# Keep-Passion/ImageStitch

Hardware: AMD Instinct MI355X
Metric: image-pairs/sec (2048x2048 grayscale, SURF+BF) (higher is better)
Workload: dtype f32

## Files before the change

### imagestitch_amd/_lib.py

```python
import ctypes as C
import os

import numpy as np

_HERE = os.path.dirname(os.path.abspath(__file__))
LIB_PATH = os.path.abspath(os.environ["VFSMS_LIB"]) if os.environ.get("VFSMS_LIB") else os.path.join(_HERE, "lib", "libvfsms.so")

VFSMS_OK = 0
VFSMS_ERR_BAD_ARG, VFSMS_ERR_CAPACITY, VFSMS_ERR_UNSUPPORTED = -1, -2, -6
ATTEMPT_INTS = 8


class VfsmsError(RuntimeError):
    pass


class SurfParams(C.Structure):
    _fields_ = [("hessian_threshold", C.c_float), ("n_octaves", C.c_int32), ("n_octave_layers", C.c_int32),
                ("extended", C.c_int32), ("upright", C.c_int32)]


class OrbParams(C.Structure):
    _fields_ = [("n_features", C.c_int32), ("scale_factor", C.c_float), ("n_levels", C.c_int32), ("edge_threshold", C.c_int32),
                ("first_level", C.c_int32), ("wta_k", C.c_int32), ("score_type", C.c_int32), ("patch_size", C.c_int32),
# ... 42 lines not shown
    "vfsms_ctx_sync": (C.c_int, [C.c_void_p]),
    "vfsms_ctx_sync_uploads": (C.c_int, [C.c_void_p]),
    "vfsms_ctx_stream": (C.c_void_p, [C.c_void_p]),
    "vfsms_ctx_set_keypoint_capacity": (C.c_int, [C.c_void_p, C.c_int]),
    "vfsms_ctx_set_offset_estimator": (C.c_int, [C.c_void_p, C.c_int, C.c_int]),
    "vfsms_ctx_set_offset_verifier": (C.c_int, [C.c_void_p, C.c_int, C.c_double, C.c_int]),
    "vfsms_ctx_set_phase_resolver": (C.c_int, [C.c_void_p, C.c_int, C.c_int, C.c_double, C.c_int]),
    "vfsms_attempt_phase_resolve_batch": (C.c_int, [C.c_void_p, C.POINTER(RoiPair), C.c_int, C.c_int, C.c_double, C.c_int, C.c_void_p, C.c_void_p, C.c_void_p]),
    "vfsms_phase_resolve_u8": (C.c_int, [C.c_void_p, C.c_void_p, C.c_void_p, C.c_int, C.c_int, C.c_int, C.c_int, C.c_int, C.c_double, C.c_int,
                                         C.c_void_p, C.c_void_p, C.c_void_p]),
    "vfsms_verify_ncc": (C.c_int, [C.c_void_p, C.c_void_p, C.c_int, C.c_void_p, C.c_int, C.c_int, C.c_int, C.c_int, C.c_int, C.c_int, C.c_void_p]),
    "vfsms_ncc_search_batch": (C.c_int, [C.c_void_p, C.POINTER(NccJob), C.c_int, C.c_int, C.c_int, C.c_void_p, C.c_void_p]),
    "vfsms_profile_enable": (C.c_int, [C.c_void_p, C.c_int]),
    "vfsms_profile_read": (C.c_int, [C.c_void_p, C.c_char_p, C.c_int, C.c_void_p, C.c_void_p, C.c_int, C.POINTER(C.c_int), C.c_int]),
    "vfsms_tile_upload": (C.c_int, [C.c_void_p, C.c_void_p, C.c_int, C.c_int, C.c_int, C.POINTER(C.c_int64)]),
    "vfsms_tile_upload_async": (C.c_int, [C.c_void_p, C.c_void_p, C.c_int, C.c_int, C.c_int, C.POINTER(C.c_int64)]),
    "vfsms_tile_reserve": (C.c_int, [C.c_void_p, C.c_int, C.c_int, C.POINTER(C.c_int64)]),
    "vfsms_tile_fill": (C.c_int, [C.c_void_p, C.c_int64, C.c_void_p, C.c_int]),
    "vfsms_tile_reserve_ch": (C.c_int, [C.c_void_p, C.c_int, C.c_int, C.c_int, C.POINTER(C.c_int64)]),
    "vfsms_tile_fill_pair": (C.c_int, [C.c_void_p, C.c_int64, C.c_int64, C.c_void_p, C.c_int, C.c_int]),
    "vfsms_tile_fill_jpeg": (C.c_int, [C.c_void_p, C.c_int64, C.c_int64, C.c_char_p, C.c_size_t]),
    "vfsms_jpeg_decode": (C.c_int, [C.c_char_p, C.c_size_t, C.c_int, C.c_void_p, C.c_size_t, C.POINTER(C.c_int), C.POINTER(C.c_int), C.POINTER(C.c_int)]),
    "vfsms_jpeg_encode": (C.c_int, [C.c_void_p, C.c_int, C.c_int, C.c_int, C.c_int, C.c_int, C.c_int, C.c_void_p, C.c_size_t, C.POINTER(C.c_size_t)]),
    "vfsms_jpeg_header": (C.c_int, [C.c_int, C.c_int, C.c_int, C.c_int, C.c_int, C.c_void_p, C.c_size_t, C.POINTER(C.c_size_t)]),
    "vfsms_jpeg_encode_device": (C.c_int, [C.c_void_p, C.c_void_p, C.c_int, C.c_int, C.c_int, C.c_int, C.c_int, C.c_int, C.c_int, C.c_void_p, C.c_size_t, C.POINTER(C.c_size_t)]),
    "vfsms_canvas_encode_jpeg_rows": (C.c_int, [C.c_void_p, C.c_int64, C.c_int, C.c_int, C.c_int, C.c_int, C.c_void_p, C.c_size_t, C.POINTER(C.c_size_t)]),
    "vfsms_jpeg_join": (C.c_int, [C.POINTER(C.c_void_p), C.POINTER(C.c_size_t), C.c_int, C.c_int, C.c_int, C.c_void_p, C.c_size_t, C.POINTER(C.c_size_t)]),
    "vfsms_canvas_blend_tile_resident": (C.c_int, [C.c_void_p, C.c_int64, C.c_int64, C.c_int, C.c_int, C.c_int, C.c_int, C.c_int, C.c_int, C.c_int]),
    "vfsms_host_alloc": (C.c_int, [C.c_void_p, C.c_size_t, C.POINTER(C.c_void_p)]),
    "vfsms_host_free": (C.c_int, [C.c_void_p, C.c_void_p]),
    "vfsms_tile_wrap": (C.c_int, [C.c_void_p, C.c_void_p, C.c_int, C.c_int, C.c_int, C.POINTER(C.c_int64)]),
    "vfsms_tile_free": (C.c_int, [C.c_void_p, C.c_int64]),
    "vfsms_integral_u8_i32": (C.c_int, [C.c_void_p, C.c_void_p, C.c_int, C.c_int, C.c_int, C.c_void_p]),
    "vfsms_surf_detect_describe": (C.c_int, [C.c_void_p, C.c_void_p, C.c_int, C.c_int, C.c_int, C.POINTER(SurfParams),
                                             C.c_void_p, C.c_void_p, C.c_void_p, C.c_int, C.POINTER(C.c_int)]),
    "vfsms_surf_detect": (C.c_int, [C.c_void_p, C.c_void_p, C.c_int, C.c_int, C.c_int, C.POINTER(SurfParams),
                                    C.c_void_p, C.c_int, C.POINTER(C.c_int)]),
    "vfsms_orb_detect_describe": (C.c_int, [C.c_void_p, C.c_void_p, C.c_int, C.c_int, C.c_int, C.POINTER(OrbParams),
                                            C.c_void_p, C.c_void_p, C.c_void_p, C.c_int, C.POINTER(C.c_int)]),
    "vfsms_sift_detect_describe": (C.c_int, [C.c_void_p, C.c_void_p, C.c_int, C.c_int, C.c_int, C.POINTER(SiftParams),
                                             C.c_void_p, C.c_void_p, C.c_void_p, C.c_int, C.POINTER(C.c_int)]),
    "vfsms_sift_pyramid": (C.c_int, [C.c_void_p, C.c_void_p, C.c_int, C.c_int, C.c_int, C.POINTER(SiftParams),
                                     C.c_void_p, C.c_void_p, C.c_size_t, C.c_void_p, C.c_int, C.POINTER(C.c_int)]),
    "vfsms_attempt_orb_batch": (C.c_int, [C.c_void_p, C.POINTER(RoiPair), C.c_int, C.POINTER(OrbParams), C.c_int, C.c_int, C.c_void_p]),
    "vfsms_attempt_sift_batch": (C.c_int, [C.c_void_p, C.POINTER(RoiPair), C.c_int, C.POINTER(SiftParams), C.c_double, C.c_int, C.c_void_p]),
    "vfsms_bf_l2_knn2_ratio": (C.c_int, [C.c_void_p, C.c_void_p, C.c_int, C.c_void_p, C.c_int, C.c_int, C.c_double,
                                         C.c_void_p, C.c_int, C.POINTER(C.c_int)]),
    "vfsms_bf_l2_knn2": (C.c_int, [C.c_void_p, C.c_void_p, C.c_int, C.c_void_p, C.c_int, C.c_int,
                                   C.c_void_p, C.c_void_p, C.c_void_p]),
    "vfsms_bf_hamming_nn": (C.c_int, [C.c_void_p, C.c_void_p, C.c_int, C.c_void_p, C.c_int, C.c_int, C.c_int,
                                      C.c_void_p, C.c_int, C.POINTER(C.c_int)]),
    "vfsms_mode_offset": (C.c_int, [C.c_void_p, C.c_void_p, C.c_int, C.c_void_p, C.c_int, C.c_void_p, C.c_int,
                                    C.c_int, C.c_void_p]),
    "vfsms_consensus_offset": (C.c_int, [C.c_void_p, C.c_void_p, C.c_int, C.c_void_p, C.c_int, C.c_void_p, C.c_int,
                                         C.c_int, C.c_int, C.c_void_p]),
    "vfsms_phase_correlate_u8": (C.c_int, [C.c_void_p, C.c_void_p, C.c_void_p, C.c_int, C.c_int, C.c_int, C.c_int,
                                           C.c_void_p]),
    "vfsms_fuse_fade_i64": (C.c_int, [C.c_void_p, C.c_void_p, C.c_void_p, C.c_int, C.c_int, C.c_int, C.c_int, C.c_int,
                                      C.c_void_p, C.c_void_p]),
    "vfsms_fuse_ramps_i64": (C.c_int, [C.c_void_p, C.c_void_p, C.c_int, C.c_int, C.c_int, C.c_int, C.c_int, C.c_int,
                                       C.c_void_p, C.c_void_p]),
    "vfsms_attempt_surf_batch": (C.c_int, [C.c_void_p, C.POINTER(RoiPair), C.c_int, C.POINTER(SurfParams), C.c_double,
                                           C.c_int, C.c_void_p]),
    "vfsms_attempt_surf_batch_enhanced": (C.c_int, [C.c_void_p, C.POINTER(RoiPair), C.c_int, C.POINTER(SurfParams), C.c_double,
                                                    C.c_int, C.c_int, C.c_double, C.c_int, C.c_void_p]),
    "vfsms_features_surf": (C.c_int, [C.c_void_p, C.c_int64, C.c_int, C.c_int, C.c_int, C.c_int, C.POINTER(SurfParams), C.c_int, C.c_double,
# ... 272 lines not shown
                                                  1 if asynchronous else 0, C.byref(h)))
        if asynchronous:
            self.__dict__.setdefault("_inflight", []).append(img)
        return self._note_tile(h.value, img.shape)

    def pinned_empty(self, shape, dtype=np.uint8):
        n = int(np.prod(shape)) * np.dtype(dtype).itemsize
        p = C.c_void_p()
        self._check(self.lib.vfsms_host_alloc(self.ctx, C.c_size_t(max(n, 1)), C.byref(p)))
        self.__dict__.setdefault("_pinned", []).append(p.value)
        buf = (C.c_uint8 * max(n, 1)).from_address(p.value)
        return np.frombuffer(buf, dtype=dtype, count=int(np.prod(shape))).reshape(shape)

    def tile_wrap(self, device_ptr, h, w, stride):
        hd = C.c_int64()
        self._check(self.lib.vfsms_tile_wrap(self.ctx, C.c_void_p(int(device_ptr)), int(h), int(w), int(stride), C.byref(hd)))
        return self._note_tile(hd.value, (int(h), int(w)))

    def tile_free(self, handle):
        self._check(self.lib.vfsms_tile_free(self.ctx, C.c_int64(handle)))
        self.__dict__.get("_shapes", {}).pop(("tile", handle), None)

    def _note_tile(self, handle, shape):
        self.__dict__.setdefault("_shapes", {})[("tile", handle)] = tuple(int(v) for v in shape)
        return handle

    def integral(self, img):
        img = _u8_2d(img)
        h, w = img.shape
        out = np.empty((h + 1, w + 1), np.int32)
        self._check(self.lib.vfsms_integral_u8_i32(self.ctx, _ptr(img), h, w, img.strides[0], _ptr(out)))
        return out

    @staticmethod
    def surf_params(hessian=100.0, n_octaves=4, n_layers=3, extended=False, upright=False):
        return SurfParams(float(hessian), int(n_octaves), int(n_layers), int(bool(extended)), int(bool(upright)))

    def surf_detect_describe(self, img, params=None, cap=None, full=False):
        img = _u8_2d(img)
        h, w = img.shape
        params = params or self.surf_params()
        cap = cap or (h * w // 24 + 4096)
        d = 128 if params.extended else 64
        kxy = np.empty((cap, 2), np.float32)
        desc = np.empty((cap, d), np.float32)
        kfull = np.empty(cap, KP_DTYPE) if full else None
        n = C.c_int()
        self._check(self.lib.vfsms_surf_detect_describe(self.ctx, _ptr(img), h, w, img.strides[0], C.byref(params),
                                                        _ptr(kxy), _ptr(desc), _ptr(kfull), cap, C.byref(n)))
        n = n.value
        if full:
            return kxy[:n].copy(), desc[:n].copy(), kfull[:n].copy()
        return kxy[:n].copy(), desc[:n].copy()

    def surf_detect(self, img, params=None, cap=None):
        img = _u8_2d(img)
        h, w = img.shape
        params = params or self.surf_params()
        cap = cap or (h * w // 24 + 4096)
        kfull = np.empty(cap, KP_DTYPE)
        n = C.c_int()
        self._check(self.lib.vfsms_surf_detect(self.ctx, _ptr(img), h, w, img.strides[0], C.byref(params),
                                               _ptr(kfull), cap, C.byref(n)))
        return kfull[:n.value].copy()

    @staticmethod
# ... 707 lines not shown
```

### imagestitch_amd/csrc/api.hip

```cpp
#include "common.h"
#include "phase_resolve_math.h"
#include <math.h>
#include <stdarg.h>
#include <stdio.h>
#include <string.h>
#include <algorithm>
#include <map>
#include <tuple>

int fuse_i64_device(vfsms_ctx *ctx, const long long *dA, const long long *dB, int r, int c, int ch, int dx, int dy,
                    uint8_t *d_out, int32_t *info, int method = 0, int levels = 4, int seam_blend = 0, int32_t *d_seam = nullptr);

static thread_local char g_err[512] = "";
void vfsms_set_error(const char *fmt, ...)
{
    va_list ap;
    va_start(ap, fmt);
    vsnprintf(g_err, sizeof(g_err), fmt, ap);
    va_end(ap);
}
extern "C" int vfsms_last_error(char *buf, int buflen)
{
    if (!buf || buflen <= 0) return VFSMS_ERR_BAD_ARG;
    snprintf(buf, (size_t)buflen, "%s", g_err);
// ... 642 lines not shown
}
int ctx_copy_small(vfsms_ctx *ctx, const void *src, size_t bytes, void *d)
{
    const size_t need = ctx->pinned_off + bytes;
    if (need > ctx->pinned.bytes()) {
        TRY(ctx->pinned.reserve(need, ctx->stream, std::max<size_t>(4 * need, (size_t)1 << 20) - need));
        ctx->pinned_off = 0;
    }
    char *stage = ctx->pinned.as<char>() + ctx->pinned_off;
    memcpy(stage, src, bytes);
    HIP_TRY(hipMemcpyAsync(d, stage, bytes, hipMemcpyHostToDevice, ctx->stream));
    ctx->pinned_off += (bytes + 255) & ~(size_t)255;
    return VFSMS_OK;
}

extern "C" int vfsms_integral_u8_i32(vfsms_ctx *ctx, const uint8_t *img, int h, int w, int stride, int32_t *sum_out)
{
    CTX_ENTER(ctx);
    if (!img || !sum_out || h <= 0 || w <= 0 || stride < w) { vfsms_set_error("integral: bad arguments"); return VFSMS_ERR_BAD_ARG; }
    const size_t sbytes = sizeof(int32_t) * (size_t)(h + 1) * (w + 1);
    TRY(ctx_arena_reserve(ctx, (size_t)h * w + sbytes + integral_carry_bytes(h, w) + 8192));
    RoiDev R; memset(&R, 0, sizeof(R));
    uint8_t *d_img;
    TRY(upload_image(ctx, img, h, w, stride, &d_img));
    R.img = d_img; R.stride = w; R.h = h; R.w = w;
    R.sum = (int32_t *)ctx_arena_alloc(ctx, sbytes);
    R.ipitch = (w + 3) & ~3;
    R.icarry = (int32_t *)ctx_arena_alloc(ctx, integral_carry_bytes(h, w));
    if (!R.sum || !R.icarry) { vfsms_set_error("arena exhausted (integral)"); return VFSMS_ERR_CAPACITY; }
    RoiDev *d_R;
    TRY(upload_array(ctx, &R, 1, &d_R));
    TRY(launch_integral(ctx, d_R, 1, h, w));
    HIP_TRY(hipMemcpyAsync(sum_out, R.sum, sbytes, hipMemcpyDeviceToHost, ctx->stream));
    HIP_TRY(hipStreamSynchronize(ctx->stream));
    return VFSMS_OK;
}

void surf_run_layout(ArenaWalk &a, SurfRun *run, const SurfSrc *S, int n, const vfsms_surf_params *p, const SurfEnh &enh)
{
    run->R.resize(n); run->E.resize(enh.mode ? n : 0);
    run->cblock = a.take<int>(16 * (size_t)n);
    for (int i = 0; i < n; i++) {
        const uint8_t *px = S[i].p; int stride = S[i].stride;
        if (enh.mode) {
            enhance_layout(a, &run->E[i], px, stride, S[i].h, S[i].w, enh.mode, enh.tile_grid);
            px = run->E[i].dst; stride = S[i].w;
        }
        surf_roi_layout(a, &run->R[i], px, stride, S[i].h, S[i].w, S[i].cap, p);
        run->R[i].counters = run->cblock ? run->cblock + 16 * i : nullptr;
    }
    run->dR = a.take<RoiDev>(n);
    run->dE = enh.mode ? a.take<EnhJob>(n) : nullptr;
}
static size_t surf_run_bytes(const SurfSrc *S, int n, const vfsms_surf_params *p, const SurfEnh &enh, int split = 0)
{
    ArenaWalk a; SurfRun run; DescWork W;
    surf_run_layout(a, &run, S, n, p, enh);
    size_t cap0 = 0, cap1 = 0;
    for (int i = 0; i < n; i++) (i < split ? cap0 : cap1) += (size_t)S[i].cap;
    if (split > 0) surf_describe_layout(a, &W, cap0);
    if (split < n) surf_describe_layout(a, &W, cap1);
    return a.off;
}
static int surf_run_carve(vfsms_ctx *ctx, SurfRun *run, const SurfSrc *S, int n, const vfsms_surf_params *p, const SurfEnh &enh)
{
    ArenaWalk a = ctx_arena_walk(ctx);
// ... 1728 lines not shown
```

### imagestitch_amd/csrc/common.h

```cpp
#pragma once
#include <hip/hip_runtime.h>
#include <stdint.h>
#include <condition_variable>
#include <list>
#include <mutex>
#include <string>
#include <unordered_map>
#include <vector>
#include "../../include/vfsms.h"
#include "arena_walk.h"
#include "device_buf.h"

#define VFSMS_MAX_LAYERS 32
#define VFSMS_MAX_WIN 768

#define VFSMS_MAX_OCTAVES 8
#ifdef __HIPCC__
__host__ __device__
#endif
constexpr int vfsms_haar_corner(int size, int k, int c)
{
    constexpr int src[10][4] = { {0, 2, 3, 7}, {3, 2, 6, 7}, {6, 2, 9, 7}, {2, 0, 7, 3}, {2, 3, 7, 6}, {2, 6, 7, 9},
                                 {1, 1, 4, 4}, {5, 1, 8, 4}, {1, 5, 4, 8}, {5, 5, 8, 8} };
    return (2 * size * src[k][c] + 9) / 18;
// ... 167 lines not shown
struct ProfScope {
    vfsms_ctx *c; int r;
    ProfScope(vfsms_ctx *ctx, const char *name) : c(ctx), r(prof_begin(ctx, name)) {}
    ~ProfScope() { prof_end(c, r); }
};

int ctx_arena_reserve(vfsms_ctx *ctx, size_t bytes);
void *ctx_arena_alloc(vfsms_ctx *ctx, size_t bytes, size_t align = 256);
ArenaWalk ctx_arena_walk(vfsms_ctx *ctx);
int ctx_arena_commit(vfsms_ctx *ctx, const ArenaWalk &a, const char *what);
int ctx_prepare_surf(vfsms_ctx *ctx, const vfsms_surf_params *p);

struct ShapeRun { int first, count, h, w; };
template <typename Rec>
static std::vector<ShapeRun> shape_runs(const Rec *recs, int n)
{
    std::vector<ShapeRun> runs;
    for (int r = 0; r < n; r++) {
        if (!runs.empty() && runs.back().h == recs[r].h && runs.back().w == recs[r].w) runs.back().count++;
        else runs.push_back(ShapeRun{r, 1, recs[r].h, recs[r].w});
    }
    return runs;
}

void surf_roi_layout(ArenaWalk &a, RoiDev *r, const uint8_t *img, int stride, int h, int w, int cap, const vfsms_surf_params *p);
struct DescWork { int *tickets; DescPlan *plan; DescRec *rec_big, *rec_small; };
void surf_describe_layout(ArenaWalk &a, DescWork *d, size_t capsum);
int launch_integral(vfsms_ctx *ctx, const RoiDev *d_rois, int nrois, int maxh, int maxw);
size_t integral_carry_bytes(int h, int w);
int launch_surf_detect(vfsms_ctx *ctx, const RoiDev *d_rois, const RoiDev *h_rois, int nrois,
                       const vfsms_surf_params *p);
int launch_surf_describe(vfsms_ctx *ctx, const RoiDev *d_rois, const RoiDev *h_rois, int nrois,
                         const vfsms_surf_params *p);
void match_layout(ArenaWalk &a, MatchDev *m, int capq, int dim, int nsplit);
void match_filter_layout(ArenaWalk &a, MatchDev *m, int capq, int capt, int cns);
int launch_max_norm2_d64(vfsms_ctx *ctx, const float *a, int n, unsigned *d_out);
int launch_bf_l2_filtered(vfsms_ctx *ctx, const MatchDev *d_jobs, int njobs, int capq, int capt, int cns);
int launch_bf_l2(vfsms_ctx *ctx, const MatchDev *d_jobs, int njobs, int capq, int nsplit, int dim);
#define BFI_PAD_NORM 0x3fffffff
struct PackJob { const float *src; const int *n_ptr; int8_t *dst; int *nrm; };
int launch_pack_i8_d128(vfsms_ctx *ctx, const PackJob *d_jobs, int njobs, int max_rows);
int launch_bf_i8_d128(vfsms_ctx *ctx, const MatchDev *d_jobs, int njobs, int capq, int nsplit);
int launch_bf_hamming(vfsms_ctx *ctx, const MatchDev *d_jobs, int njobs, int capq, int nsplit, int max_dist);
enum MatchTailKind {
    TAIL_VOTE,
    TAIL_PAIRS,
    TAIL_KNN,
    TAIL_GIVEN_PAIRS
};
struct MatchTail {
    MatchTailKind kind;
    double ratio;
    int max_dist;
    int offset_evaluate;
    bool merged = false;
    int estimator = VFSMS_OFFSET_MODE, tol = 0;
};
int launch_match_tail(vfsms_ctx *ctx, const MatchDev *d_jobs, int njobs, int capq, const MatchTail &tail);
int launch_consensus(vfsms_ctx *ctx, const MatchDev *d_jobs, int njobs, int capq, int tol, int offset_evaluate);
int launch_verify(vfsms_ctx *ctx, const MatchDev *d_jobs, int njobs, double threshold, int min_pixels);
#define VFSMS_ADJUST_MAX_RADIUS 16
struct AdjJob { const uint8_t *a, *b; int sa, sb, h, w, dx, dy; };
size_t adjust_sums_bytes(int njobs, int radius);
int launch_adjust_search(vfsms_ctx *ctx, const AdjJob *d_jobs, const AdjJob *h_jobs, int njobs, int radius, int min_pixels,
                         unsigned long long *d_sums, int32_t *d_best4, int32_t *d_surface);
int ctx_prepare_orb(vfsms_ctx *ctx, const vfsms_orb_params *p);
// ... 124 lines not shown
```

### imagestitch_amd/csrc/surf_kernels.hip

```cpp
#include "common.h"
#include "detmath.h"
#include <math.h>
#include <float.h>
#include <string.h>
#include <stdlib.h>
#include <algorithm>
#include <vector>

#define GAS __attribute__((address_space(1)))
typedef GAS const uint8_t *g_cu8;
typedef GAS const int32_t *g_ci32;
typedef GAS float *g_f32;
typedef GAS const float *g_cf32;
typedef GAS int32_t *g_i32;
__device__ __forceinline__ int cv_round_f(float v) { return (int)rintf(v); }
__device__ __forceinline__ uint8_t round_u8_pos(float v) { return (uint8_t)__float_as_uint(v + 12582912.f); }
__device__ __forceinline__ int cv_round_d(double v) { return (int)rint(v); }
__device__ __forceinline__ int cv_floor_d(double v) { return (int)floor(v); }
__device__ __forceinline__ int cv_ceil_d(double v) { return (int)ceil(v); }

__device__ __forceinline__ int wave_incl_scan(int v)
{
    const int lane = threadIdx.x & 63;
#pragma unroll
    for (int d = 1; d < 64; d <<= 1) {
        int n = __shfl_up(v, d, 64);
        if (lane >= d) v += n;
    }
    return v;
}

#define INT_TH 16
typedef int int4u __attribute__((ext_vector_type(4), aligned(4)));
typedef uint32_t u32u __attribute__((aligned(1)));
// ... 907 lines not shown
            if (nvalid[q] == 0) {
                if (lane == 0) R.kps[k].size = -1.f;
            } else {
                float bm = mod_s[q][lane]; int bi = lane;
                if (!(bm > 0.f)) bm = 0.f;
                if (lane < 8) { float m2 = mod_s[q][64 + lane]; if (m2 > bm) { bm = m2; bi = 64 + lane; } }
#pragma unroll
                for (int off = 32; off >= 1; off >>= 1) {
                    const float om = __shfl_xor(bm, off, 64); const int oi = __shfl_xor(bi, off, 64);
                    if (om > bm || (om == bm && oi < bi)) { bm = om; bi = oi; }
                }
                if (lane == 0) {
                    float bestx = 0, besty = 0;
                    if (bm > 0.f) { bestx = sx_s[q][bi]; besty = sy_s[q][bi]; }
                    R.kps[k].angle = fast_atan2_deg(-besty, bestx);
                }
            }
        }
    }
}

#ifdef VFSMS_DESC_TIMING
__device__ unsigned long long g_desc_cycles[8];
#define DT_MARK(ph) do { if (threadIdx.x == 0) { unsigned long long _n = clock64(); atomicAdd(&g_desc_cycles[ph], _n - _t0); _t0 = _n; } } while (0)
#define DT_START unsigned long long _t0 = clock64()
extern "C" int vfsms_debug_desc_cycles(unsigned long long *out) { return hipMemcpyFromSymbol(out, HIP_SYMBOL(g_desc_cycles), sizeof(unsigned long long) * 8) == hipSuccess ? 0 : -3; }
__device__ unsigned long long g_desc_trips[4];
#define DT_TRIP(n) do {} while (0)
__device__ unsigned long long g_desc_unit_cycles[4];
#define DT_UNIT_BEGIN unsigned long long _u0 = clock64()
#define DT_UNIT_END(n) do { _uacc[n] += clock64() - _u0; _ucnt[n]++; } while (0)
extern "C" int vfsms_debug_desc_unit_cycles(unsigned long long *out) { return hipMemcpyFromSymbol(out, HIP_SYMBOL(g_desc_unit_cycles), sizeof(unsigned long long) * 4) == hipSuccess ? 0 : -3; }
extern "C" int vfsms_debug_desc_trips(unsigned long long *out) { return hipMemcpyFromSymbol(out, HIP_SYMBOL(g_desc_trips), sizeof(unsigned long long) * 4) == hipSuccess ? 0 : -3; }
#else
#define DT_MARK(ph) do {} while (0)
#define DT_START do {} while (0)
#define DT_TRIP(n) do {} while (0)
#define DT_UNIT_BEGIN do {} while (0)
#define DT_UNIT_END(n) do {} while (0)
#endif
#ifndef VFSMS_EXP
#define VFSMS_EXP 0
#endif
#ifndef DESC_WBUF
#define DESC_WBUF 15360
#endif
__device__ __forceinline__ void origin_chain(float *row, float s, const float d, const int n)
{
    int i = 0;
    for (; i + 4 <= n; i += 4) {
        const float a = s, b = a + d, c = b + d, e = c + d;
        s = e + d;
        row[i] = a; row[i + 1] = b; row[i + 2] = c; row[i + 3] = e;
    }
    for (; i < n; i++, s += d) row[i] = s;
}

struct WinGeom {
    int win; float sin_dir, cos_dir;
    int h, w, stride; g_cu8 img;
    g_cu8 pair;
    int upright, usx, usy;
};

__device__ __forceinline__ int win_sample_xy(const WinGeom &G, double px, double py)
{
    const int ncols1 = G.w - 1, nrows1 = G.h - 1;
    const int ix = (int)px, iy = (int)py;
    if (px >= 0.0 && py >= 0.0 && ix < ncols1 && iy < nrows1) {
        const float a = (float)__builtin_amdgcn_fract(px), b = (float)__builtin_amdgcn_fract(py);
        g_cu8 p = G.img + (size_t)iy * G.stride + ix;
        const float v = p[0] * (1.f - a) * (1.f - b) + p[1] * a * (1.f - b) + p[G.stride] * (1.f - a) * b + p[G.stride + 1] * a * b;
        return (int)(uint8_t)cv_round_f(v);
    }
    const int x = min(max(cv_round_d(px), 0), ncols1);
    const int y = min(max(cv_round_d(py), 0), nrows1);
    return (int)G.img[(size_t)y * G.stride + x];
}
__device__ __forceinline__ int win_sample_upright(const WinGeom &G, int i, int j)
{
    const int x = min(max(G.usx + i, 0), G.w - 1);
    const int y = min(max(G.usy - j, 0), G.h - 1);
    return (int)G.img[(size_t)y * G.stride + x];
}

typedef float float2v __attribute__((ext_vector_type(2)));
__device__ __forceinline__ float bilinear_pk(uint32_t top, float a, float b)
{
    const float na = 1.f - a, nb = 1.f - b;
// ... 220 lines not shown
__device__ __forceinline__ uint8_t area_out(const float sum, const int mode, const float inv_area)
{
    if (mode == 2) return (uint8_t)(((int)sum + 2) >> 2);
    if (mode == 1) return sat_u8(sum * inv_area);
    return sat_u8(sum);
}
__device__ __forceinline__ uint8_t area_col_tab(const float *rb, const AreaRec &c, const int mode, const float inv_area)
{
    float sum = c.a0 * rb[0];
    for (int t = 1; t < c.n; t++) sum += (t < c.n - 1 ? c.af : c.al) * rb[t * 21];
    return area_out(sum, mode, inv_area);
}
#define DESC_ACC_OFF (DESC_WBUF - 441 * 4)
#define DESC_PASS 36

__device__ void describe_one(const RoiDev &R, const SurfTables *T, const AreaRec *area_tab, const DescRec &rec, int extended, int upright, const int band)
{
    DT_START;
    const int k = rec.k;
    __shared__ float sx_row[VFSMS_MAX_WIN], sy_row[VFSMS_MAX_WIN];
    __shared__ uint8_t PATCH[21][21 + 3];
    __shared__ AreaRec REC[AREA_RECS];
    __shared__ uint8_t WINBUF[DESC_WBUF];
    __shared__ float rowsum[40 * 21];
    __shared__ uint8_t STRIP_IN[VFSMS_MAX_WIN / 8 + 8];
    WinGeom G;
    G.win = max(21, min(rec.win, VFSMS_MAX_WIN));
    G.h = R.h; G.w = R.w; G.stride = R.stride; G.img = (g_cu8)R.img; G.pair = (g_cu8)R.pair;
    G.upright = upright; G.usx = 0; G.usy = 0; G.sin_dir = rec.sin_dir; G.cos_dir = rec.cos_dir;
    const int win = G.win;
    const int dsz = 21;
    if (threadIdx.x < AREA_RECS * 8) ((int *)REC)[threadIdx.x] = ((const int *)(area_tab + (size_t)win * AREA_RECS))[threadIdx.x];
    __syncthreads();
    const int nmin = __builtin_amdgcn_readfirstlane(REC[21].j0), nmax = __builtin_amdgcn_readfirstlane(REC[21].n);
    const int mode = __builtin_amdgcn_readfirstlane(REC[21].mode);
    const float inv_area = REC[21].a0;
    if (!upright) {
        if (threadIdx.x == 0 || threadIdx.x == 64) {
            const float sin_dir = rec.sin_dir, cos_dir = rec.cos_dir;
            const float win_offset = -(float)(win - 1) / 2;
            const int need = band >= 0 ? min(win, REC[band].j0 + REC[band].n) : win;
            if (threadIdx.x == 0) origin_chain(sx_row, rec.x + win_offset * cos_dir + win_offset * sin_dir, sin_dir, need);
            else origin_chain(sy_row, rec.y - win_offset * sin_dir + win_offset * cos_dir, cos_dir, need);
        }
    } else {
        const float win_offset = -(float)(win - 1) / 2;
        G.usx = cv_round_f(rec.x + win_offset);
        G.usy = cv_round_f(rec.y - win_offset);
    }
    __syncthreads();
    DT_MARK(0);

    const bool tail_ok = nmax - max(nmin - 1, 1) <= AREA_TAIL;
    auto reduce_rows = [&](const int st_lo, int dyA, const int dy_stop) {
        while (dyA < dy_stop) {
            const int lo = REC[dyA].j0;
            int dyB = dyA + 1;
            while (dyB < dy_stop && REC[dyB].j0 + REC[dyB].n - lo <= 40) dyB++;
            const int nr = REC[dyB - 1].j0 + REC[dyB - 1].n - lo;
            for (int e = threadIdx.x; e < nr * 21; e += 256) {
                const int r = (int)(((uint32_t)e * 3121u) >> 16), dx = e - 21 * r;
                if (tail_ok) {
                    const AreaRec cx = REC[dx];
                    float w[AREA_TAIL];
                    area_tail_weights(cx, nmin, w);
                    rowsum[e] = area_row_tab_w(WINBUF + (lo - st_lo + r) * win, cx, nmin, nmax, w);
                } else
                    rowsum[e] = area_row_tab(WINBUF + (lo - st_lo + r) * win, REC[dx], nmin, nmax);
            }
            __syncthreads();
            for (int o = threadIdx.x; o < (dyB - dyA) * 21; o += 256) {
                const int dyl = (int)(((uint32_t)o * 3121u) >> 16), dx = o - 21 * dyl;
                const AreaRec ry = REC[dyA + dyl];
                PATCH[dyA + dyl][dx] = area_col_tab(rowsum + (ry.j0 - lo) * 21 + dx, ry, mode, inv_area);
            }
            __syncthreads();
// ... 165 lines not shown
        rec.cos_dir = (float)cd;
    }
    (cls < 3 ? big : small)[plan->seg_base[roi][cls] + idx] = rec;
}

__global__ __launch_bounds__(ORI_KP * 128, 8) void k_orientation(const RoiDev *rois, const SurfTables *T, int upright)
{
    const RoiDev &R = rois[blockIdx.y];
    const int n = min(R.counters[0], R.cap);
    const int k0 = blockIdx.x * ORI_KP;
    if (k0 >= n) return;
    orientation_block(R, T, k0, n, upright);
}

#define DESC_SMALL_WIN 64
struct SmallLds { uint8_t win[DESC_SMALL_WIN * DESC_SMALL_WIN + 64]; float sx[DESC_SMALL_WIN + 8], sy[DESC_SMALL_WIN + 8]; AreaRec rec[AREA_RECS]; int rec_win; uint8_t strip_in[DESC_SMALL_WIN / 8 + 8]; };

__device__ __forceinline__ void wave_sync_lds()
{
    __builtin_amdgcn_fence(__ATOMIC_ACQ_REL, "wavefront");
    __builtin_amdgcn_wave_barrier();
}

__device__ void describe_small(const RoiDev &R, const AreaRec *area_tab, const DescRec &rec, int upright, SmallLds &L)
{
    const int lane = threadIdx.x & 63;
    const int k = rec.k;
    WinGeom G;
    G.win = min(rec.win, DESC_SMALL_WIN);
    G.h = R.h; G.w = R.w; G.stride = R.stride; G.img = (g_cu8)R.img; G.pair = (g_cu8)R.pair;
    G.upright = upright; G.usx = 0; G.usy = 0; G.sin_dir = rec.sin_dir; G.cos_dir = rec.cos_dir;
    const int win = G.win;
    const int dsz = 21;
    if (L.rec_win != win) {
        wave_sync_lds();
        const int *src = (const int *)(area_tab + (size_t)max(win, dsz) * AREA_RECS);
        for (int e = lane; e < AREA_RECS * 8; e += 64) ((int *)L.rec)[e] = src[e];
        if (lane == 0) L.rec_win = win;
    }
    if (!upright) {
        const float sin_dir = rec.sin_dir, cos_dir = rec.cos_dir;
        if (lane < 2) {
            const float win_offset = -(float)(win - 1) / 2;
            const float sx0 = rec.x + win_offset * cos_dir + win_offset * sin_dir, sy0 = rec.y - win_offset * sin_dir + win_offset * cos_dir;
            origin_chain(lane == 0 ? L.sx : L.sy, lane == 0 ? sx0 : sy0, lane == 0 ? sin_dir : cos_dir, win);
        }
    } else {
        const float win_offset = -(float)(win - 1) / 2;
        G.usx = cv_round_f(rec.x + win_offset);
        G.usy = cv_round_f(rec.y - win_offset);
    }
    wave_sync_lds();
    stage_rows<1>(G, L.sx, L.sy, 0, win, L.win, L.strip_in);
    wave_sync_lds();
    const int nmin = __builtin_amdgcn_readfirstlane(L.rec[21].j0), nmax = __builtin_amdgcn_readfirstlane(L.rec[21].n);
    const int mode = __builtin_amdgcn_readfirstlane(L.rec[21].mode);
    const float inv_area = L.rec[21].a0;
    const bool tail_ok = nmax - max(nmin - 1, 1) <= AREA_TAIL;
    uint8_t *prow = R.patch + (size_t)k * VFSMS_PATCH_ROW;
    for (int o = lane; o < dsz * dsz; o += 64) {
        const int dy = (int)(((uint32_t)o * 3121u) >> 16), dx = o - dsz * dy;
        const AreaRec ry = L.rec[dy], rx = L.rec[dx];
        const uint8_t *S = L.win + ry.j0 * win;
        float sum;
        if (tail_ok) {
            float w[AREA_TAIL];
            area_tail_weights(rx, nmin, w);
            sum = ry.a0 * area_row_tab_w(S, rx, nmin, nmax, w);
            for (int ty = 1; ty < nmax; ty++) {
                const float beta = ty < ry.n - 1 ? ry.af : (ty == ry.n - 1 ? ry.al : 0.f);
                sum += beta * area_row_tab_w(S + ty * win, rx, nmin, nmax, w);
            }
        } else {
            sum = ry.a0 * area_row_tab(S, rx, nmin, nmax);
            for (int ty = 1; ty < nmax; ty++) {
                const float beta = ty < ry.n - 1 ? ry.af : (ty == ry.n - 1 ? ry.al : 0.f);
                sum += beta * area_row_tab(S + ty * win, rx, nmin, nmax);
            }
        }
        uint8_t outv;
        if (mode == 2) outv = (uint8_t)(((int)sum + 2) >> 2);
        else if (mode == 1) outv = sat_u8(sum * inv_area);
        else outv = sat_u8(sum);
        prow[o] = outv;
    }
    wave_sync_lds();
}

#ifndef DESC_SMALL_WGS
#define DESC_SMALL_WGS 7
#endif
__device__ __forceinline__ DescRec load_rec_uniform(const DescRec *p)
{
    const int *q = (const int *)p;
    DescRec r;
    r.roi = __builtin_amdgcn_readfirstlane(q[0]); r.k = __builtin_amdgcn_readfirstlane(q[1]);
    r.win = __builtin_amdgcn_readfirstlane(q[2]); r.pad = 0;
    r.sin_dir = __int_as_float(__builtin_amdgcn_readfirstlane(q[4])); r.cos_dir = __int_as_float(__builtin_amdgcn_readfirstlane(q[5]));
    r.x = __int_as_float(__builtin_amdgcn_readfirstlane(q[6])); r.y = __int_as_float(__builtin_amdgcn_readfirstlane(q[7]));
    return r;
}
__global__ __launch_bounds__(256, DESC_SMALL_WGS) void k_describe_small(const RoiDev *rois, const DescPlan *plan, const DescRec *recs, int *counter,
                                                                 const AreaRec *area_tab, int upright)
{
    __shared__ SmallLds L[4];
    if (threadIdx.x < 4) L[threadIdx.x].rec_win = -1;
    __syncthreads();
    const int lane = threadIdx.x & 63, wave = __builtin_amdgcn_readfirstlane((int)(threadIdx.x >> 6));
    int head = 0;
    for (;;) {
        int slot = -1;
        if (lane == 0)
            while (head < DESC_HEADS) {
                const int q = (blockIdx.x + head) & (DESC_HEADS - 1);
                const int n = plan->small_tickets[q];
                const int t = n > 0 ? atomicAdd(counter + q * DESC_HEAD_STRIDE, 1) : 0;
                if (t < n) { slot = plan->small_start[q] + t; break; }
                head++;
            }
        slot = __builtin_amdgcn_readfirstlane(slot);
        head = __builtin_amdgcn_readfirstlane(head);
        if (slot < 0) break;
        const DescRec rec = load_rec_uniform(recs + slot);
        describe_small(rois[rec.roi], area_tab, rec, upright, L[wave]);
    }
}

__global__ __launch_bounds__(256) void k_pair_rows(const RoiDev *rois)
{
    const RoiDev &R = rois[blockIdx.z];
    const int y = blockIdx.y, x = (blockIdx.x * 256 + threadIdx.x) * 4;
    if (y >= R.h || x >= R.w) return;
    g_cu8 r0 = (g_cu8)R.img + (size_t)y * R.stride + x, r1 = (g_cu8)R.img + (size_t)min(y + 1, R.h - 1) * R.stride + x;
    GAS uint16_t *dst = (GAS uint16_t *)R.pair + (size_t)y * R.w + x;
    if (x + 4 <= R.w) {
        const uint32_t a = *(GAS const u32u *)r0, b = *(GAS const u32u *)r1;
#pragma unroll
        for (int k = 0; k < 4; k++) dst[k] = (uint16_t)(((a >> (8 * k)) & 0xff) | (((b >> (8 * k)) & 0xff) << 8));
    } else {
        for (int k = 0; x + k < R.w; k++) dst[k] = (uint16_t)(r0[k] | (r1[k] << 8));
    }
}

#ifndef DESC_WGS
#define DESC_WGS 6
#endif
__global__ __launch_bounds__(256, DESC_WGS) void k_describe(const RoiDev *rois, const DescPlan *plan, const DescRec *recs, int *counter, const SurfTables *T,
                                                  const AreaRec *area_tab, int extended, int upright)
{
    __shared__ int s_slot, s_band;
    int head = 0;
#ifdef VFSMS_DESC_TIMING
    unsigned long long tq = clock64();
#endif
    for (;;) {
        __syncthreads();
        if (threadIdx.x == 0) {
            int slot = -1, band = -1;
// ... 332 lines not shown
```

### include/vfsms.h

```cpp
#ifndef VFSMS_H
#define VFSMS_H
#include <stdint.h>

#ifdef __cplusplus
extern "C" {
#endif

#define VFSMS_OK 0
#define VFSMS_ERR_BAD_ARG (-1)
#define VFSMS_ERR_CAPACITY (-2)
#define VFSMS_ERR_HIP (-3)
#define VFSMS_ERR_FFT (-4)
#define VFSMS_ERR_NO_DEVICE (-5)
#define VFSMS_ERR_UNSUPPORTED (-6)

typedef struct vfsms_ctx vfsms_ctx;

typedef struct {
    float x, y, size, angle, response;
    int32_t octave, class_id;
} vfsms_keypoint;

typedef struct {
    float hessian_threshold;
// ... 44 lines not shown
#define VFSMS_PHASE_RESOLVE_NCC 1
#define VFSMS_PHASE_MAX_PEAKS 8
int vfsms_ctx_set_phase_resolver(vfsms_ctx *ctx, int resolver, int peaks, double threshold, int min_pixels);

int vfsms_profile_enable(vfsms_ctx *ctx, int on);
int vfsms_profile_read(vfsms_ctx *ctx, char *names, int names_len, double *ms, int64_t *calls, int cap,
                       int *n_out, int reset);

int vfsms_tile_upload(vfsms_ctx *ctx, const uint8_t *img, int h, int w, int stride, int64_t *handle);
int vfsms_tile_upload_async(vfsms_ctx *ctx, const uint8_t *img, int h, int w, int stride, int64_t *handle);
int vfsms_tile_upload_ch(vfsms_ctx *ctx, const uint8_t *img, int h, int w, int ch, int stride_bytes, int async, int64_t *handle);
int vfsms_tile_reserve(vfsms_ctx *ctx, int h, int w, int64_t *handle);
int vfsms_tile_fill(vfsms_ctx *ctx, int64_t handle, const uint8_t *img, int stride);
int vfsms_tile_reserve_ch(vfsms_ctx *ctx, int h, int w, int ch, int64_t *handle);
#define VFSMS_SRC_GRAY8 0
#define VFSMS_SRC_YCC24 1
#define VFSMS_SRC_YCCX32 2
int vfsms_tile_fill_pair(vfsms_ctx *ctx, int64_t gray, int64_t color, const uint8_t *src, int stride_bytes, int format);
int vfsms_tile_fill_jpeg(vfsms_ctx *ctx, int64_t gray, int64_t color, const uint8_t *jpeg, size_t nbytes);
int vfsms_jpeg_decode(const uint8_t *jpeg, size_t nbytes, int want_planes, uint8_t *out, size_t cap, int *h, int *w, int *comp);
int vfsms_jpeg_encode(const uint8_t *rows, int n_rows, int cols, int channels, int stride_bytes, int bgr, int quality,
                      uint8_t *out, size_t cap, size_t *nbytes);
int vfsms_jpeg_join(const uint8_t *const *streams, const size_t *sizes, int n_stripes, int stripe_rows, int total_rows,
                    uint8_t *out, size_t cap, size_t *nbytes);
int vfsms_jpeg_header(int rows, int cols, int ch, int quality, int restart_mcus, uint8_t *out, size_t cap, size_t *nbytes);
int vfsms_jpeg_encode_device(vfsms_ctx *ctx, const uint8_t *img, int h, int w, int ch, int stride, int bgr, int quality, int restart_mcus,
                             uint8_t *out, size_t cap, size_t *nbytes);
int vfsms_host_alloc(vfsms_ctx *ctx, size_t bytes, void **ptr);
int vfsms_host_free(vfsms_ctx *ctx, void *ptr);
int vfsms_tile_wrap(vfsms_ctx *ctx, const void *device_ptr, int h, int w, int stride, int64_t *handle);
int vfsms_tile_free(vfsms_ctx *ctx, int64_t handle);

int vfsms_integral_u8_i32(vfsms_ctx *ctx, const uint8_t *img, int h, int w, int stride, int32_t *sum_out);

int vfsms_surf_detect_describe(vfsms_ctx *ctx, const uint8_t *img, int h, int w, int stride,
                               const vfsms_surf_params *params,
                               float *kps_xy, float *desc, vfsms_keypoint *kps_full,
                               int cap, int *n_out);
int vfsms_surf_detect(vfsms_ctx *ctx, const uint8_t *img, int h, int w, int stride,
                      const vfsms_surf_params *params, vfsms_keypoint *kps_full, int cap, int *n_out);

int vfsms_orb_detect_describe(vfsms_ctx *ctx, const uint8_t *img, int h, int w, int stride,
                              const vfsms_orb_params *params,
                              float *kps_xy, uint8_t *desc, vfsms_keypoint *kps_full, int cap, int *n_out);

int vfsms_sift_detect_describe(vfsms_ctx *ctx, const uint8_t *img, int h, int w, int stride, const vfsms_sift_params *params,
                               float *kps_xy, float *desc, vfsms_keypoint *kps_full, int cap, int *n_out);
int vfsms_sift_pyramid(vfsms_ctx *ctx, const uint8_t *img, int h, int w, int stride, const vfsms_sift_params *params,
                       float *gauss, float *dog, size_t cap_floats, int32_t *shapes, int shapes_cap, int *n_octaves);

int vfsms_bf_l2_knn2_ratio(vfsms_ctx *ctx, const float *q, int nq, const float *t, int nt, int dim,
                           double ratio, int32_t *pairs, int cap, int *m_out);
int vfsms_bf_l2_knn2(vfsms_ctx *ctx, const float *q, int nq, const float *t, int nt, int dim,
                     int32_t *idx1, float *d1, float *d2);
int vfsms_bf_hamming_nn(vfsms_ctx *ctx, const uint8_t *q, int nq, const uint8_t *t, int nt, int nbytes,
                        int max_dist, int32_t *pairs, int cap, int *m_out);

int vfsms_mode_offset(vfsms_ctx *ctx, const float *kpsA, int nA, const float *kpsB, int nB,
                      const int32_t *pairs, int m, int offset_evaluate, int32_t *out4);
int vfsms_consensus_offset(vfsms_ctx *ctx, const float *kpsA, int nA, const float *kpsB, int nB,
                           const int32_t *pairs, int m, int tol_px, int offset_evaluate, int32_t *out4);

int vfsms_verify_ncc(vfsms_ctx *ctx, const uint8_t *a, int a_stride, const uint8_t *b, int b_stride, int h, int w,
                     int dx, int dy, int min_pixels, int64_t *out8);

typedef struct { int64_t tile_a, tile_b; int32_t dx, dy; } vfsms_ncc_job;
// ... 136 lines not shown
```

Measured before the change: 2497.

## Parallelize SURF sample-origin chain across wavefront lanes with speculative verification

```diff
diff --git a/imagestitch_amd/_lib.py b/imagestitch_amd/_lib.py
--- a/imagestitch_amd/_lib.py
+++ b/imagestitch_amd/_lib.py
@@ -98,6 +98,7 @@
     "vfsms_tile_wrap": (C.c_int, [C.c_void_p, C.c_void_p, C.c_int, C.c_int, C.c_int, C.POINTER(C.c_int64)]),
     "vfsms_tile_free": (C.c_int, [C.c_void_p, C.c_int64]),
     "vfsms_integral_u8_i32": (C.c_int, [C.c_void_p, C.c_void_p, C.c_int, C.c_int, C.c_int, C.c_void_p]),
+    "vfsms_surf_row_origins": (C.c_int, [C.c_void_p, C.c_void_p, C.c_void_p, C.c_void_p, C.c_int, C.c_void_p, C.c_int]),
     "vfsms_surf_detect_describe": (C.c_int, [C.c_void_p, C.c_void_p, C.c_int, C.c_int, C.c_int, C.POINTER(SurfParams),
                                              C.c_void_p, C.c_void_p, C.c_void_p, C.c_int, C.POINTER(C.c_int)]),
     "vfsms_surf_detect": (C.c_int, [C.c_void_p, C.c_void_p, C.c_int, C.c_int, C.c_int, C.POINTER(SurfParams),
@@ -436,6 +437,13 @@
         self._check(self.lib.vfsms_integral_u8_i32(self.ctx, _ptr(img), h, w, img.strides[0], _ptr(out)))
         return out
 
+    def surf_row_origins(self, s0, d, n):
+        s0 = np.ascontiguousarray(s0, np.float32); d = np.ascontiguousarray(d, np.float32); n = np.ascontiguousarray(n, np.int32)
+        assert s0.ndim == 1 and s0.shape == d.shape == n.shape
+        out = np.empty((len(n), max(int(n.max()), 1)), np.float32)
+        self._check(self.lib.vfsms_surf_row_origins(self.ctx, _ptr(s0), _ptr(d), _ptr(n), len(n), _ptr(out), out.shape[1]))
+        return out
+
     @staticmethod
     def surf_params(hessian=100.0, n_octaves=4, n_layers=3, extended=False, upright=False):
         return SurfParams(float(hessian), int(n_octaves), int(n_layers), int(bool(extended)), int(bool(upright)))
diff --git a/imagestitch_amd/csrc/api.hip b/imagestitch_amd/csrc/api.hip
--- a/imagestitch_amd/csrc/api.hip
+++ b/imagestitch_amd/csrc/api.hip
@@ -698,6 +698,27 @@
     TRY(upload_array(ctx, &R, 1, &d_R));
     TRY(launch_integral(ctx, d_R, 1, h, w));
     HIP_TRY(hipMemcpyAsync(sum_out, R.sum, sbytes, hipMemcpyDeviceToHost, ctx->stream));
+    HIP_TRY(hipStreamSynchronize(ctx->stream));
+    return VFSMS_OK;
+}
+
+extern "C" int vfsms_surf_row_origins(vfsms_ctx *ctx, const float *s0, const float *d, const int *n, int count, float *out, int pitch)
+{
+    CTX_ENTER(ctx);
+    if (!s0 || !d || !n || !out || count <= 0 || pitch <= 0) { vfsms_set_error("row origins: bad arguments"); return VFSMS_ERR_BAD_ARG; }
+    for (int c = 0; c < count; c++)
+        if (n[c] < 0 || n[c] > pitch) { vfsms_set_error("row origins: a chain is longer than the pitch"); return VFSMS_ERR_BAD_ARG; }
+    const size_t obytes = sizeof(float) * (size_t)count * pitch;
+    TRY(ctx_arena_reserve(ctx, obytes + 3 * sizeof(float) * (size_t)count + 8192));
+    float *d_s0, *d_d, *d_out; int *d_n;
+    TRY(upload_array(ctx, s0, count, &d_s0));
+    TRY(upload_array(ctx, d, count, &d_d));
+    TRY(upload_array(ctx, n, count, &d_n));
+    d_out = (float *)ctx_arena_alloc(ctx, obytes);
+    if (!d_out) { vfsms_set_error("arena exhausted (row origins)"); return VFSMS_ERR_CAPACITY; }
+    HIP_TRY(hipMemsetAsync(d_out, 0, obytes, ctx->stream));
+    TRY(launch_row_origins(ctx, d_s0, d_d, d_n, count, d_out, pitch));
+    HIP_TRY(hipMemcpyAsync(out, d_out, obytes, hipMemcpyDeviceToHost, ctx->stream));
     HIP_TRY(hipStreamSynchronize(ctx->stream));
     return VFSMS_OK;
 }
diff --git a/imagestitch_amd/csrc/common.h b/imagestitch_amd/csrc/common.h
--- a/imagestitch_amd/csrc/common.h
+++ b/imagestitch_amd/csrc/common.h
@@ -223,6 +223,7 @@
                        const vfsms_surf_params *p);
 int launch_surf_describe(vfsms_ctx *ctx, const RoiDev *d_rois, const RoiDev *h_rois, int nrois,
                          const vfsms_surf_params *p);
+int launch_row_origins(vfsms_ctx *ctx, const float *d_s0, const float *d_d, const int *d_n, int count, float *d_out, int pitch);
 void match_layout(ArenaWalk &a, MatchDev *m, int capq, int dim, int nsplit);
 void match_filter_layout(ArenaWalk &a, MatchDev *m, int capq, int capt, int cns);
 int launch_max_norm2_d64(vfsms_ctx *ctx, const float *a, int n, unsigned *d_out);
diff --git a/imagestitch_amd/csrc/origin_chain.h b/imagestitch_amd/csrc/origin_chain.h
--- /dev/null
+++ b/imagestitch_amd/csrc/origin_chain.h
@@ -0,0 +1,75 @@
+#pragma once
+#include <stdint.h>
+
+#ifdef __HIPCC__
+#define OC_HD __host__ __device__
+#else
+#define OC_HD
+#endif
+
+#define OC_LANES 64
+
+OC_HD inline void origin_chain(float *row, float s, const float d, const int n)
+{
+    int i = 0;
+    for (; i + 4 <= n; i += 4) {
+        const float a = s, b = a + d, c = b + d, e = c + d;
+        s = e + d;
+        row[i] = a; row[i + 1] = b; row[i + 2] = c; row[i + 3] = e;
+    }
+    for (; i < n; i++, s += d) row[i] = s;
+}
+
+OC_HD inline uint32_t oc_bits(const float v)
+{
+    uint32_t u;
+    __builtin_memcpy(&u, &v, sizeof(u));
+    return u;
+}
+
+template <typename W>
+OC_HD inline int origin_chain_fill(const W &w, float *row, const float s0, const float d, const int n)
+{
+    int b = 0, trips = 0;
+    float t1 = s0;
+    while (b < n) {
+        const float t2 = t1 + d;
+        const double D = (double)t2 - (double)t1;
+        typename W::template reg<float> cur, step;
+        typename W::template reg<int> bad;
+        for (int l = w.lane_begin(); l < w.lane_end(); l++) {
+            const float nxt = l == 0 ? t2 : (float)((double)t1 + (double)(l + 1) * D);
+            cur[l] = l == 0 ? t1 : l == 1 ? t2 : (float)((double)t1 + (double)l * D);
+            step[l] = cur[l] + d;
+            bad[l] = oc_bits(step[l]) != oc_bits(nxt);
+        }
+        const unsigned long long m = w.ballot(bad);
+        const int f = m ? __builtin_ctzll(m) : OC_LANES;
+        for (int l = w.lane_begin(); l < w.lane_end(); l++)
+            if (l <= f && b + l < n) row[b + l] = cur[l];
+        const int last = f < OC_LANES - 1 ? f : OC_LANES - 1;
+        t1 = w.read_lane(step, last);
+        b += last + 1;
+        trips++;
+    }
+    return trips;
+}
+
+#ifdef __HIPCC__
+struct OcDeviceWave {
+    template <typename T> struct reg {
+        T v;
+        __device__ __forceinline__ T &operator[](int) { return v; }
+        __device__ __forceinline__ const T &operator[](int) const { return v; }
+    };
+    int lane;
+    __device__ __forceinline__ OcDeviceWave() : lane((int)(threadIdx.x & (OC_LANES - 1))) {}
+    __device__ __forceinline__ int lane_begin() const { return lane; }
+    __device__ __forceinline__ int lane_end() const { return lane + 1; }
+    __device__ __forceinline__ unsigned long long ballot(const reg<int> &p) const { return __ballot(p.v); }
+    __device__ __forceinline__ float read_lane(const reg<float> &r, const int l) const
+    {
+        return __int_as_float(__builtin_amdgcn_readlane(__float_as_int(r.v), l));
+    }
+};
+#endif
diff --git a/imagestitch_amd/csrc/surf_kernels.hip b/imagestitch_amd/csrc/surf_kernels.hip
--- a/imagestitch_amd/csrc/surf_kernels.hip
+++ b/imagestitch_amd/csrc/surf_kernels.hip
@@ -1,5 +1,6 @@
 #include "common.h"
 #include "detmath.h"
+#include "origin_chain.h"
 #include <math.h>
 #include <float.h>
 #include <string.h>
@@ -973,6 +974,8 @@
 #define DT_UNIT_END(n) do { _uacc[n] += clock64() - _u0; _ucnt[n]++; } while (0)
 extern "C" int vfsms_debug_desc_unit_cycles(unsigned long long *out) { return hipMemcpyFromSymbol(out, HIP_SYMBOL(g_desc_unit_cycles), sizeof(unsigned long long) * 4) == hipSuccess ? 0 : -3; }
 extern "C" int vfsms_debug_desc_trips(unsigned long long *out) { return hipMemcpyFromSymbol(out, HIP_SYMBOL(g_desc_trips), sizeof(unsigned long long) * 4) == hipSuccess ? 0 : -3; }
+__device__ unsigned long long g_desc_small_cycles[4];
+extern "C" int vfsms_debug_desc_small_cycles(unsigned long long *out) { return hipMemcpyFromSymbol(out, HIP_SYMBOL(g_desc_small_cycles), sizeof(unsigned long long) * 4) == hipSuccess ? 0 : -3; }
 #else
 #define DT_MARK(ph) do {} while (0)
 #define DT_START do {} while (0)
@@ -986,16 +989,6 @@
 #ifndef DESC_WBUF
 #define DESC_WBUF 15360
 #endif
-__device__ __forceinline__ void origin_chain(float *row, float s, const float d, const int n)
-{
-    int i = 0;
-    for (; i + 4 <= n; i += 4) {
-        const float a = s, b = a + d, c = b + d, e = c + d;
-        s = e + d;
-        row[i] = a; row[i + 1] = b; row[i + 2] = c; row[i + 3] = e;
-    }
-    for (; i < n; i++, s += d) row[i] = s;
-}
 
 struct WinGeom {
     int win; float sin_dir, cos_dir;
@@ -1282,16 +1275,18 @@
     const int dsz = 21;
     if (threadIdx.x < AREA_RECS * 8) ((int *)REC)[threadIdx.x] = ((const int *)(area_tab + (size_t)win * AREA_RECS))[threadIdx.x];
     __syncthreads();
+    DT_MARK(7);
     const int nmin = __builtin_amdgcn_readfirstlane(REC[21].j0), nmax = __builtin_amdgcn_readfirstlane(REC[21].n);
     const int mode = __builtin_amdgcn_readfirstlane(REC[21].mode);
     const float inv_area = REC[21].a0;
     if (!upright) {
-        if (threadIdx.x == 0 || threadIdx.x == 64) {
+        const int wv = __builtin_amdgcn_readfirstlane((int)(threadIdx.x >> 6));
+        if (wv < 2) {
             const float sin_dir = rec.sin_dir, cos_dir = rec.cos_dir;
             const float win_offset = -(float)(win - 1) / 2;
-            const int need = band >= 0 ? min(win, REC[band].j0 + REC[band].n) : win;
-            if (threadIdx.x == 0) origin_chain(sx_row, rec.x + win_offset * cos_dir + win_offset * sin_dir, sin_dir, need);
-            else origin_chain(sy_row, rec.y - win_offset * sin_dir + win_offset * cos_dir, cos_dir, need);
+            const int need = band >= 0 ? min(win, __builtin_amdgcn_readfirstlane(REC[band].j0 + REC[band].n)) : win;
+            const float sx0 = rec.x + win_offset * cos_dir + win_offset * sin_dir, sy0 = rec.y - win_offset * sin_dir + win_offset * cos_dir;
+            origin_chain_fill(OcDeviceWave(), wv == 0 ? sx_row : sy_row, wv == 0 ? sx0 : sy0, wv == 0 ? sin_dir : cos_dir, need);
         }
     } else {
         const float win_offset = -(float)(win - 1) / 2;
@@ -1523,12 +1518,18 @@
     G.upright = upright; G.usx = 0; G.usy = 0; G.sin_dir = rec.sin_dir; G.cos_dir = rec.cos_dir;
     const int win = G.win;
     const int dsz = 21;
+#ifdef VFSMS_DESC_TIMING
+    const unsigned long long _w0 = clock64();
+#endif
     if (L.rec_win != win) {
         wave_sync_lds();
         const int *src = (const int *)(area_tab + (size_t)max(win, dsz) * AREA_RECS);
         for (int e = lane; e < AREA_RECS * 8; e += 64) ((int *)L.rec)[e] = src[e];
         if (lane == 0) L.rec_win = win;
     }
+#ifdef VFSMS_DESC_TIMING
+    const unsigned long long _w1 = clock64();
+#endif
     if (!upright) {
         const float sin_dir = rec.sin_dir, cos_dir = rec.cos_dir;
         if (lane < 2) {
@@ -1542,6 +1543,9 @@
         G.usy = cv_round_f(rec.y - win_offset);
     }
     wave_sync_lds();
+#ifdef VFSMS_DESC_TIMING
+    const unsigned long long _w2 = clock64();
+#endif
     stage_rows<1>(G, L.sx, L.sy, 0, win, L.win, L.strip_in);
     wave_sync_lds();
     const int nmin = __builtin_amdgcn_readfirstlane(L.rec[21].j0), nmax = __builtin_amdgcn_readfirstlane(L.rec[21].n);
@@ -1576,6 +1580,12 @@
         prow[o] = outv;
     }
     wave_sync_lds();
+#ifdef VFSMS_DESC_TIMING
+    if (lane == 0) {
+        atomicAdd(&g_desc_small_cycles[0], _w1 - _w0); atomicAdd(&g_desc_small_cycles[1], _w2 - _w1);
+        atomicAdd(&g_desc_small_cycles[2], clock64() - _w0); atomicAdd(&g_desc_small_cycles[3], 1ull);
+    }
+#endif
 }
 
 #ifndef DESC_SMALL_WGS
@@ -1615,6 +1625,21 @@
         const DescRec rec = load_rec_uniform(recs + slot);
         describe_small(rois[rec.roi], area_tab, rec, upright, L[wave]);
     }
+}
+
+__global__ __launch_bounds__(64) void k_row_origins(const float *s0, const float *d, const int *n, float *out, int pitch)
+{
+    const int c = blockIdx.x;
+    const int len = min(max(__builtin_amdgcn_readfirstlane(n[c]), 0), pitch);
+    const float s = __int_as_float(__builtin_amdgcn_readfirstlane(__float_as_int(s0[c])));
+    const float dd = __int_as_float(__builtin_amdgcn_readfirstlane(__float_as_int(d[c])));
+    origin_chain_fill(OcDeviceWave(), out + (size_t)c * pitch, s, dd, len);
+}
+int launch_row_origins(vfsms_ctx *ctx, const float *d_s0, const float *d_d, const int *d_n, int count, float *d_out, int pitch)
+{
+    hipLaunchKernelGGL(k_row_origins, dim3(count), dim3(64), 0, ctx->stream, d_s0, d_d, d_n, d_out, pitch);
+    HIP_TRY(hipGetLastError());
+    return VFSMS_OK;
 }
 
 __global__ __launch_bounds__(256) void k_pair_rows(const RoiDev *rois)
diff --git a/include/vfsms.h b/include/vfsms.h
--- a/include/vfsms.h
+++ b/include/vfsms.h
@@ -100,6 +100,8 @@
 int vfsms_tile_free(vfsms_ctx *ctx, int64_t handle);
 
 int vfsms_integral_u8_i32(vfsms_ctx *ctx, const uint8_t *img, int h, int w, int stride, int32_t *sum_out);
+
+int vfsms_surf_row_origins(vfsms_ctx *ctx, const float *s0, const float *d, const int *n, int count, float *out, int pitch);
 
 int vfsms_surf_detect_describe(vfsms_ctx *ctx, const uint8_t *img, int h, int w, int stride,
                                const vfsms_surf_params *params,
```

Result: no change. 2509 (median of 2 runs) (+0.5%).
